# josef-w/Differentiable-iLQR

Measured on AMD Instinct MI355X. Metric: iLQR iters/sec (whole node), batch=65536 cartpole T=25 at 1/2/4/8 MI355X, higher is better.
Workload: dtype f32; 1 GPU; cartpole n=5 m=1 T=25, unconstrained iLQR, 65536 problems per GPU, step = one whole-batch MPC solve of lqr_iter=10 from u=0; batch_per_gpu=65536, global_batch=65536, T=25, lqr_iter=10, parallelism=batch-sharded x1 (no collective)

## Files before the change

### differentiable-ilqr_amd/csrc/dilqr_fused.h

```cpp
#pragma once
#include "dilqr_common.h"
#include "dilqr_launch.h"

namespace dilqr {

constexpr int TRAJ_AOS = 0, TRAJ_REC = 1;

template <int TL, int n, int m>
DEV void ld_xu(float (&x)[n], float (&u)[m], const float* __restrict__ xp, const float* __restrict__ up, size_t t,
               int B, int b) {
  const size_t tb = t * B + b;
  if constexpr (TL == TRAJ_REC) {
    float r[n + m];
    ld(r, (xp + (size_t)b * (n + m)) + t * (size_t)B * (n + m));
#pragma unroll
    for (int i = 0; i < n; ++i) x[i] = r[i];
#pragma unroll
    for (int a = 0; a < m; ++a) u[a] = r[n + a];
  } else {
    ld(x, xp + tb * n);
    ld(u, up + tb * m);
  }
}

template <int TL, int n, int m>
DEV void st_xu(float* __restrict__ xp, float* __restrict__ up, const float (&x)[n], const float (&u)[m], size_t t,
               int B, int b) {
  const size_t tb = t * B + b;
  if constexpr (TL == TRAJ_REC) {
    float r[n + m];
#pragma unroll
    for (int i = 0; i < n; ++i) r[i] = x[i];
#pragma unroll
    for (int a = 0; a < m; ++a) r[n + a] = u[a];
    st(xp + tb * (n + m), r);
  } else {
    st(xp + tb * n, x);
    st(up + tb * m, u);
  }
}

template <int d>
struct CostFull {
  static constexpr bool kDiag = false;
  static constexpr bool kSym = false;
  const float* __restrict__ C;
  const float* __restrict__ c;
  DEV void load(float (&Cr)[d][d], float (&cr)[d], size_t t, int B, int b) const {
    const size_t tb = t * B + b;
    ld2(Cr, C + tb * d * d); ld(cr, c + tb * d);
  }
};

template <int d>
constexpr int packed_cost_floats() { return d * (d + 1) / 2 + d; }
template <int d>
constexpr bool packed_diag_ok() { return (2 * d) % 4 == 0; }

constexpr unsigned char kCostSym = 1, kCostDiag = 2, kCostTinv = 4;

template <int d>
DEV void pack_cost(const float (&C)[d][d], const float (&c)[d], float (&buf)[packed_cost_floats<d>()], bool& sym,
                   bool& diag) {
  int k = 0;
#pragma unroll
  for (int i = 0; i < d; ++i) buf[k++] = C[i][i];
#pragma unroll
  for (int i = 0; i < d; ++i) buf[k++] = c[i];
  unsigned asym = 0u, offd = 0u;
#pragma unroll
  for (int i = 0; i < d; ++i)
#pragma unroll
    for (int j = i + 1; j < d; ++j) {
      asym |= __float_as_uint(C[i][j]) ^ __float_as_uint(C[j][i]);
      offd |= __float_as_uint(C[i][j]) | __float_as_uint(C[j][i]);
      buf[k++] = C[i][j];
    }
  sym &= asym == 0u;
  diag &= offd == 0u;
}

template <int K>
DEV bool same_bits(const float (&a)[K], const float (&b)[K]) {
  unsigned dif = 0u;
#pragma unroll
  for (int k = 0; k < K; ++k) dif |= __float_as_uint(a[k]) ^ __float_as_uint(b[k]);
  return dif == 0u;
}

template <int d, bool DIAG = false, bool TINV = false>
struct CostPacked {
  static constexpr bool kDiag = DIAG;
  static constexpr bool kSym = true;
  const float* __restrict__ P;
  int T;
  DEV void load(float (&Cr)[d][d], float (&cr)[d], size_t t_, int B, int b) const {
    constexpr int PK = packed_cost_floats<d>();
    const size_t t = TINV ? (size_t)(T - 1) : t_;
    if constexpr (DIAG) {
      static_assert(packed_diag_ok<d>(), "diagonal read needs whole float4 planes");
      constexpr int Q4 = SoaRec<PK>::Q4;
      const float4* q = reinterpret_cast<const float4*>(P);
      float buf[2 * d];
#pragma unroll
      for (int j = 0; j < 2 * d / 4; ++j) {
        float4 v = q[(t * Q4 + j) * B + b];
        buf[4 * j] = v.x; buf[4 * j + 1] = v.y; buf[4 * j + 2] = v.z; buf[4 * j + 3] = v.w;
      }
      const float z = 0.f;
#pragma unroll
      for (int i = 0; i < d; ++i) {
#pragma unroll
        for (int j = 0; j < d; ++j) Cr[i][j] = z;
        Cr[i][i] = buf[i];
        cr[i] = buf[d + i];
      }
    } else {
      float buf[PK];
      SoaRec<PK>::load(buf, P, T, t, B, b);
      int k = 2 * d;
#pragma unroll
      for (int i = 0; i < d; ++i) {
        Cr[i][i] = buf[i];
        cr[i] = buf[d + i];
      }
#pragma unroll
      for (int i = 0; i < d; ++i)
#pragma unroll
        for (int j = i + 1; j < d; ++j) { Cr[i][j] = buf[k]; Cr[j][i] = buf[k]; ++k; }
    }
  }
};

template <int d>
struct CostDiagConst {
  static constexpr bool kDiag = true;
  static constexpr bool kSym = true;
  float dg[d], cc[d];
  DEV void init(const float* __restrict__ P, int T, int B, int b) {
    float Cr[d][d], cr[d];
    CostPacked<d, true>{P, T}.load(Cr, cr, T - 1, B, b);
#pragma unroll
    for (int i = 0; i < d; ++i) { dg[i] = Cr[i][i]; cc[i] = cr[i]; }
  }
  template <int PK>
  DEV void set(const float (&pk)[PK]) {
#pragma unroll
    for (int i = 0; i < d; ++i) { dg[i] = pk[i]; cc[i] = pk[d + i]; }
  }
  DEV void load(float (&Cr)[d][d], float (&cr)[d], size_t, int, int) const {
    const float z = 0.f;
#pragma unroll
    for (int i = 0; i < d; ++i) {
#pragma unroll
      for (int j = 0; j < d; ++j) Cr[i][j] = z;
      Cr[i][i] = dg[i];
      cr[i] = cc[i];
    }
  }
};

template <int m, int BM>
struct StepBounds {
  float lo[m], hi[m];
  DEV void load(const Bounds& bd, int t, int B, int b) {
    if constexpr (BM == DILQR_BOUNDS_TENSOR) {
      const size_t tb = (size_t)t * B + b;
      ld(lo, bd.lo_t + tb * m); ld(hi, bd.hi_t + tb * m);
    }
  }
  DEV float l(const Bounds& bd, int a) const {
    if constexpr (BM == DILQR_BOUNDS_TENSOR) return lo[a];
    else return bd.lo;
  }
  DEV float h(const Bounds& bd, int a) const {
    if constexpr (BM == DILQR_BOUNDS_TENSOR) return hi[a];
    else return bd.hi;
  }
};

template <int n, int m, int TL, int BM>
struct SweepIn {
  static constexpr int d = n + m;
  float C[d][d], c[d], x[n], u[m];
  StepBounds<m, BM> bnd;
  template <class CostT>
  DEV void load(const CostT& cs, const float* __restrict__ xp, const float* __restrict__ up, const Bounds& bd, int t,
                int B, int b) {
    cs.load(C, c, t, B, b); ld_xu<TL>(x, u, xp, up, t, B, b); bnd.load(bd, t, B, b);
  }
};

struct GainRecs {
  float* p;
  int B, b;
};

template <int n, int m, int GREC, int TL, int BM>
struct FwdIn {
  static constexpr int d = n + m;
  float g[GREC], u[m], C[d][d], c[d], xnext[n], unext[m];
  StepBounds<m, BM> bnd;
  template <class CostT>
  DEV void load(const GainRecs& gr, const float* __restrict__ up, const CostT& cs,
                const float* __restrict__ xp, const Bounds& bd, int T, int t, int t1, int B, int b) {
    SoaRec<GREC>::load(g, gr.p, T, t, gr.B, gr.b); cs.load(C, c, t, B, b); bnd.load(bd, t, B, b);
    if constexpr (TL == TRAJ_REC) {
      ld_xu<TL>(xnext, unext, xp, up, t1, B, b);
    } else {
      ld(u, up + ((size_t)t * B + b) * m);
      ld(xnext, xp + ((size_t)t1 * B + b) * n);
    }
  }
};

#ifndef DILQR_PF
#define DILQR_PF 2
#endif
constexpr int kPF = DILQR_PF;
#ifndef DILQR_PF_LS
#define DILQR_PF_LS 1
#endif
constexpr int kPFL = DILQR_PF_LS;
static_assert(kPFL == 1 || kPFL == 2, "the line search prefetches one or two steps ahead");

#ifndef DILQR_PHASE_SKIP
#define DILQR_PHASE_SKIP 0
#endif

template <class Model, int BM, int TL, class CostT, bool PAIR = false>
DEV int line_search(int T, int B, int b, const Model md, const float* __restrict__ x_init, const CostT& cs,
                    const float* __restrict__ x, const float* __restrict__ u, const Bounds& bd, float decay,
                    int max_ls, const GainRecs& ws, float* __restrict__ xa_out,
                    float* __restrict__ ua_out, float* __restrict__ xb_out, float* __restrict__ ub_out,
                    float* __restrict__ du_sq, float old_cost, float& cost_out, float& alpha_out,
                    bool b_in_gains = false) {
  constexpr int n = Model::N, m = Model::M, d = n + m;
  constexpr int GREC = m * n + m;
  static_assert(TL != TRAJ_REC || GREC == d, "B records in the gain slots need m = 1");
  if constexpr (PAIR) {
    max_ls = 2;
    b_in_gains = true;
  }
  float alpha = 1.f, cost = 0.f;
  int win = 0;
  for (int p = 0; p < max_ls; p += 2) {
    const bool twoB = p + 1 < max_ls;
    const float aA = alpha, aB = alpha * decay;
    const f2 al = {aA, aB};
    f2 xp[n], dp[n];
    {
      float x0[n];
      ld(x0, x_init + (size_t)b * n);
#pragma unroll
      for (int i = 0; i < n; ++i) { xp[i] = f2{x0[i], x0[i]}; dp[i] = f2{0.f, 0.f}; }
      if constexpr (TL == TRAJ_AOS) {
        st(xa_out + (size_t)b * n, x0);
        if (twoB) st(xb_out + (size_t)b * n, x0);
      }
    }
    f2 cp = {0.f, 0.f};
    auto cl = [T](int s) { return s < T ? s : T - 1; };
    FwdIn<n, m, GREC, TL, BM> cur, n1, n2;
    cur.load(ws, u, cs, x, bd, T, 0, cl(1), B, b);
    if constexpr (TL == TRAJ_REC) {
      float x0r[n];
      ld_xu<TL>(x0r, cur.u, x, u, 0, B, b);
    }
    if constexpr (kPFL >= 2) {
      if (T > 1) n1.load(ws, u, cs, x, bd, T, 1, cl(2), B, b);
    }
    auto step = [&](int t, auto last_c, auto& c, auto& nx) {
      constexpr bool LAST = decltype(last_c)::value;
      if constexpr (!LAST) {
        if constexpr (kPFL >= 2) {
          if (t + 2 < T) n2.load(ws, u, cs, x, bd, T, t + 2, cl(t + 3), B, b);
        } else {
          nx.load(ws, u, cs, x, bd, T, t + 1, cl(t + 2), B, b);
        }
      }
      f2 nu[m];
#pragma unroll
      for (int a = 0; a < m; ++a) {
        f2 sp = {0.f, 0.f};
#pragma unroll
        for (int j = 0; j < n; ++j) sp += c.g[a * n + j] * dp[j];
        nu[a] = (sp + c.u[a]) + al * c.g[m * n + a];
        if constexpr (BM != DILQR_BOUNDS_NONE) {
          const float lo = c.bnd.l(bd, a), hi = c.bnd.h(bd, a);
          nu[a] = f2{eclamp(nu[a].x, lo, hi), eclamp(nu[a].y, lo, hi)};
        }
      }
      {
        float ua[m], ub[m];
#pragma unroll
        for (int a = 0; a < m; ++a) { ua[a] = nu[a].x; ub[a] = nu[a].y; }
        if constexpr (TL == TRAJ_REC) {
          float xa[n], xb[n];
#pragma unroll
          for (int i = 0; i < n; ++i) { xa[i] = xp[i].x; xb[i] = xp[i].y; }
          st_xu<TL>(xa_out, nullptr, xa, ua, t, B, b);
          if (twoB) {
            if (b_in_gains) {
              float rb[d];
#pragma unroll
              for (int i = 0; i < n; ++i) rb[i] = xb[i];
#pragma unroll
              for (int a = 0; a < m; ++a) rb[n + a] = ub[a];
              SoaRec<d>::store(ws.p, rb, T, t, ws.B, ws.b);
            } else {
              st_xu<TL>(xb_out, nullptr, xb, ub, t, B, b);
            }
          }
        } else {
          st(ua_out + ((size_t)t * B + b) * m, ua);
          if (twoB) st(ub_out + ((size_t)t * B + b) * m, ub);
        }
      }
      if (p == 0) {
#pragma unroll
        for (int a = 0; a < m; ++a) {
          float e = c.u[a] - nu[a].x;
          du_sq[((size_t)t * m + a) * B + b] = e * e;
        }
      }
      f2 tau[d];
#pragma unroll
      for (int i = 0; i < n; ++i) tau[i] = xp[i];
#pragma unroll
      for (int a = 0; a < m; ++a) tau[n + a] = nu[a];
      cp += quad_cost<d, CostT::kDiag>(c.C, c.c, tau);
      if constexpr (!LAST) {
        f2 xnext[n];
        md.forward(xp, nu, xnext);
        float xa[n], xb[n];
#pragma unroll
        for (int i = 0; i < n; ++i) {
          dp[i] = xnext[i] - c.xnext[i];
          xp[i] = xnext[i];
          xa[i] = xnext[i].x;
          xb[i] = xnext[i].y;
        }
        if constexpr (TL == TRAJ_AOS) {
          st(xa_out + ((size_t)(t + 1) * B + b) * n, xa);
          if (twoB) st(xb_out + ((size_t)(t + 1) * B + b) * n, xb);
        }
      }
      if constexpr (!LAST) {
        if constexpr (TL == TRAJ_REC) {
#pragma unroll
          for (int a = 0; a < m; ++a) nx.u[a] = c.unext[a];
        }
      }
    };
    for (int t = 0; t < T - 1; ++t) {
      step(t, std::false_type{}, cur, n1);
      cur = n1;
      if constexpr (kPFL >= 2) n1 = n2;
    }
    step(T - 1, std::true_type{}, cur, n1);
    const float cA = cp.x, cB = cp.y;
    if (!(cA > old_cost) || p == max_ls - 1) { cost = cA; alpha = aA; win = 0; break; }
    if (!(cB > old_cost) || p + 1 == max_ls - 1) { cost = cB; alpha = aB; win = 1; break; }
    alpha = aB * decay;
  }
  if constexpr (TL == TRAJ_REC) {
    if (b_in_gains && win == 1) {
      for (int t = 0; t < T; ++t) {
        float rb[d], xt[n], ut[m];
        SoaRec<d>::load(rb, ws.p, T, t, ws.B, ws.b);
#pragma unroll
        for (int i = 0; i < n; ++i) xt[i] = rb[i];
#pragma unroll
        for (int a = 0; a < m; ++a) ut[a] = rb[n + a];
        st_xu<TL>(xb_out, nullptr, xt, ut, t, B, b);
      }
    }
  }
  cost_out = cost;
  alpha_out = alpha;
  return win;
}

template <class Model, int BM, int TL, bool ROLLOUT, class CostT, bool PREV = false>
DEV int ilqr_problem(int T, int B, int b, const Model md, const float* __restrict__ x_init, const CostT& cs,
                     float* __restrict__ pack_out, unsigned char* __restrict__ sym_out, const float* __restrict__ x,
                     const float* __restrict__ u, const Bounds& bd, float decay, int max_ls,
                     const GainRecs& ws, float* __restrict__ xa_out, float* __restrict__ ua_out,
                     float* __restrict__ xb_out, float* __restrict__ ub_out, float* __restrict__ du_sq,
                     float& cost_out, float& alpha_out, bool b_in_gains = false,
                     float prev_cost = 0.f, unsigned* flags_out = nullptr) {
  constexpr int n = Model::N, m = Model::M, d = n + m;
  constexpr int MODE = BM == DILQR_BOUNDS_NONE ? GAIN_UNC : GAIN_BOX;
  constexpr int GREC = m * n + m;
  constexpr int PK = packed_cost_floats<d>();
  float old_cost = 0.f;
  if constexpr (PREV) old_cost = prev_cost;
  bool sym = true, diag = true, tinv = true;
  bool symsofar = true;
  float pk_last[PK];
  {
    RiccatiState<n, m> rs;
    rs.init();
    float xn[n];
#pragma unroll
    for (int i = 0; i < n; ++i) xn[i] = 0.f;
    SweepIn<n, m, TL, BM> cur, n1, n2;
    cur.load(cs, x, u, bd, T - 1, B, b);
    if constexpr (kPF >= 2) n1.load(cs, x, u, bd, T > 1 ? T - 2 : 0, B, b);
    using SI = SweepIn<n, m, TL, BM>;
    auto sweep_body = [&](int t, auto last_c, const SI& cur, float (&g)[GREC]) {
      constexpr bool LAST = decltype(last_c)::value;
      float tau[d], Ctau[d], cb[d];
#pragma unroll
      for (int i = 0; i < n; ++i) tau[i] = cur.x[i];
#pragma unroll
      for (int a = 0; a < m; ++a) tau[n + a] = cur.u[a];
      if (pack_out) {
        float buf[PK];
        pack_cost(cur.C, cur.c, buf, sym, diag);
        if constexpr (LAST) {
          SoaRec<PK>::store(pack_out, buf, T, t, B, b);
#pragma unroll
          for (int k = 0; k < PK; ++k) pk_last[k] = buf[k];
        } else {
          const bool same = same_bits(buf, pk_last);
          if (tinv && !same)
            for (int s = t + 1; s < T - 1; ++s) SoaRec<PK>::store(pack_out, pk_last, T, s, B, b);
          tinv &= same;
          if (!tinv) SoaRec<PK>::store(pack_out, buf, T, t, B, b);
        }
      }
      float obj = 0.f;
      if constexpr (PREV) c_tau<d, CostT::kDiag>(cur.C, tau, Ctau);
      else obj = quad_cost<d, CostT::kDiag>(cur.C, cur.c, tau, Ctau);
#pragma unroll
      for (int i = 0; i < d; ++i) cb[i] = Ctau[i] + cur.c[i];
      float Ft[n][d];
      if constexpr (!LAST) {
        if constexpr (ROLLOUT && Model::kJacFromNext) md.jacobian_next(cur.x, cur.u, xn, Ft);
        else md.jacobian(cur.x, cur.u, Ft);
      } else {
#pragma unroll
        for (int i = 0; i < n; ++i)
#pragma unroll
          for (int j = 0; j < d; ++j) Ft[i][j] = 0.f;
      }
      float zIt[m], lb[m], ub[m];
#pragma unroll
      for (int a = 0; a < m; ++a) {
        zIt[a] = 0.f; lb[a] = 0.f; ub[a] = 0.f;
        if constexpr (MODE == GAIN_BOX) {
          lb[a] = cur.bnd.l(bd, a) - cur.u[a];
          ub[a] = cur.bnd.h(bd, a) - cur.u[a];
        }
      }
      float Kt[m][n], kt[m];
      using FS = typename Model::FSparsity;
      if constexpr (CostT::kSym) {
        rs.template step<MODE, FS, CostT::kDiag, true>(cur.C, cb, Ft, zIt, lb, ub, Kt, kt);
      } else {
        symsofar &= bitwise_symmetric(cur.C);
        if (symsofar) rs.template step<MODE, FS, CostT::kDiag, true>(cur.C, cb, Ft, zIt, lb, ub, Kt, kt);
        else rs.template step<MODE, FS, CostT::kDiag, false>(cur.C, cb, Ft, zIt, lb, ub, Kt, kt);
      }
#pragma unroll
      for (int a = 0; a < m; ++a) {
#pragma unroll
        for (int j = 0; j < n; ++j) g[a * n + j] = Kt[a][j];
        g[m * n + a] = kt[a];
      }
      if constexpr (!PREV) old_cost += obj;
#pragma unroll
      for (int i = 0; i < n; ++i) xn[i] = cur.x[i];
    };
    auto sweep_step = [&](int t, auto last_c) {
      if constexpr (kPF >= 2) n2.load(cs, x, u, bd, t > 1 ? t - 2 : 0, B, b);
      else n1.load(cs, x, u, bd, t > 0 ? t - 1 : 0, B, b);
      float g[GREC];
      sweep_body(t, last_c, cur, g);
      SoaRec<GREC>::store(ws.p, g, T, t, ws.B, ws.b);
      cur = n1;
      if constexpr (kPF >= 2) n1 = n2;
    };
    sweep_step(T - 1, std::true_type{});
#ifndef DILQR_SWEEP_UNROLL
#define DILQR_SWEEP_UNROLL 2
#endif
#pragma unroll DILQR_SWEEP_UNROLL
    for (int t = T - 2; t >= 0; --t) sweep_step(t, std::false_type{});
    if (sym_out) {
      const unsigned char f = sym ? (unsigned char)(kCostSym | (diag && packed_diag_ok<d>() ? kCostDiag : 0) |
                                                    (tinv ? kCostTinv : 0))
                                  : 0;
      sym_out[b] = f;
      if (flags_out) *flags_out = f;
    }
  }
  DILQR_STAMP(2);
#if DILQR_PHASE_SKIP & 1
  cost_out = old_cost;
  alpha_out = 1.f;
  return 0;
#endif
  if constexpr (!CostT::kDiag && packed_diag_ok<d>()) {
    if (pack_out && sym && diag && tinv) {
      CostDiagConst<d> cc;
      cc.set(pk_last);
      if (b_in_gains && max_ls == 2)
        return line_search<Model, BM, TL, CostDiagConst<d>, true>(T, B, b, md, x_init, cc, x, u, bd, decay, max_ls, ws,
                                                                  xa_out, ua_out, xb_out, ub_out, du_sq, old_cost,
                                                                  cost_out, alpha_out, b_in_gains);
      return line_search<Model, BM, TL>(T, B, b, md, x_init, cc, x, u, bd, decay, max_ls, ws, xa_out, ua_out,
                                         xb_out, ub_out, du_sq, old_cost, cost_out, alpha_out, b_in_gains);
    }
  }
  if (b_in_gains && max_ls == 2)
    return line_search<Model, BM, TL, CostT, true>(T, B, b, md, x_init, cs, x, u, bd, decay, max_ls, ws, xa_out,
                                                   ua_out, xb_out, ub_out, du_sq, old_cost, cost_out, alpha_out,
                                                   b_in_gains);
  return line_search<Model, BM, TL>(T, B, b, md, x_init, cs, x, u, bd, decay, max_ls, ws, xa_out, ua_out, xb_out,
                                     ub_out, du_sq, old_cost, cost_out, alpha_out, b_in_gains);
}

template <class Model, int BM>
__global__ void __launch_bounds__(kBlock) k_ilqr_iterate(int T, int B, const float* __restrict__ theta,
                                                         const float* __restrict__ x_init, const float* __restrict__ C,
                                                         const float* __restrict__ c, const float* __restrict__ x,
                                                         const float* __restrict__ u, Bounds bd, float decay, int max_ls,
                                                         float* __restrict__ ws, float* __restrict__ x_out,
                                                         float* __restrict__ u_out, float* __restrict__ cost_out,
                                                         float* __restrict__ du_sq, float* __restrict__ alpha_out,
                                                         const dilqr_mpc_ctrl* __restrict__ ctrl) {
  if (ctrl && ctrl->stopped) return;
  int b = blockIdx.x * blockDim.x + threadIdx.x;
  if (b >= B) return;
  constexpr int n = Model::N, m = Model::M;
  constexpr int GREC = m * n + m;
  Model md; md.load(theta);
  float cost, alpha;
  float* xb = ws + (size_t)T * B * GREC;
  float* ub = xb + (size_t)T * B * n;
  const int win = ilqr_problem<Model, BM, TRAJ_AOS, false>(T, B, b, md, x_init, CostFull<n + m>{C, c}, nullptr, nullptr, x, u,
                                                   bd, decay,
                                            max_ls, GainRecs{ws, B, b},
                                            x_out, u_out, xb, ub, du_sq, cost, alpha);
  if (win) {
    for (int t = 0; t < T; ++t) {
      const size_t tb = (size_t)t * B + b;
      float xt[n], ut[m];
      ld(xt, xb + tb * n); ld(ut, ub + tb * m);
      st(x_out + tb * n, xt); st(u_out + tb * m, ut);
    }
  }
  cost_out[b] = cost;
  alpha_out[b] = alpha;
}

using MpcState = dilqr_mpc_state;
constexpr int kSlots = 4;

DEV bool mpc_decide(const MpcState& S, int B, int k, int G, float eps, int not_improved_lim);

DEV void free_slots(int cur, int best, int& sa, int& sb) {
  sa = -1;
  sb = -1;
#pragma unroll
  for (int s = 0; s < kSlots; ++s) {
    const bool fr = s != cur && s != best;
    sb = (fr && sa >= 0 && sb < 0) ? s : sb;
    sa = (fr && sa < 0) ? s : sa;
  }
}

struct LaneIter {
  float cost, alpha;
  int slot;
};

template <class Model, int BM, bool LG, bool FIRST, bool PREV = true, int GS = kBlock>
DEV LaneIter mpc_iteration_lane(int T, int B, int b, const Model md, const float* __restrict__ x_init,
                                const float* __restrict__ C, const float* __restrict__ c, const Bounds& bd,
                                float decay, int max_ls, const MpcState& S, float* __restrict__ du_sq,
                                float* __restrict__ lds_gains, int cur, int best, unsigned pk, float prev_cost,
                                unsigned* flags_out = nullptr) {
  constexpr int n = Model::N, m = Model::M;
  const size_t TBd = (size_t)T * B * (n + m);
  int sa, sb;
  free_slots(cur, best, sa, sb);
  const float* xcur = S.Xs + cur * TBd;
  float* xsa = S.Xs + sa * TBd;
  float* xsb = S.Xs + sb * TBd;
  float cost, alpha;
  int win;
  const GainRecs gr = LG ? GainRecs{lds_gains, GS, (int)threadIdx.x} : GainRecs{S.ws, B, b};
  const CostFull<n + m> full{C, c};
  const bool b_lds = LG && max_ls <= 2;
  if constexpr (FIRST) {
    win = ilqr_problem<Model, BM, TRAJ_REC, true>(T, B, b, md, x_init, full, S.Cpk, S.Cpk ? S.cost_sym : nullptr,
                                                  xcur, nullptr, bd, decay, max_ls, gr, xsa, nullptr, xsb, nullptr,
                                                  du_sq, cost, alpha, b_lds, 0.f, flags_out);
  } else {
    if ((pk & (kCostDiag | kCostTinv)) == (kCostDiag | kCostTinv)) {
      if constexpr (packed_diag_ok<n + m>()) {
        CostDiagConst<n + m> cc;
        cc.init(S.Cpk, T, B, b);
        win = ilqr_problem<Model, BM, TRAJ_REC, true, CostDiagConst<n + m>, PREV>(T, B, b, md, x_init, cc, nullptr, nullptr, xcur, nullptr, bd,
                                                      decay, max_ls, gr, xsa, nullptr, xsb, nullptr, du_sq, cost,
                                                      alpha, b_lds, prev_cost);
      } else {
        __builtin_unreachable();
      }
#ifdef DILQR_ONLY_DIAGCONST
    } else {
      __builtin_unreachable();
    }
#else
    } else if (pk & kCostDiag) {
      if constexpr (packed_diag_ok<n + m>())
        win = ilqr_problem<Model, BM, TRAJ_REC, true, CostPacked<n + m, true>, PREV>(T, B, b, md, x_init, CostPacked<n + m, true>{S.Cpk, T}, nullptr,
                                                      nullptr, xcur, nullptr, bd, decay, max_ls, gr, xsa, nullptr, xsb,
                                                      nullptr, du_sq, cost, alpha, b_lds, prev_cost);
      else
        __builtin_unreachable();
    } else if ((pk & (kCostSym | kCostTinv)) == (kCostSym | kCostTinv))
      win = ilqr_problem<Model, BM, TRAJ_REC, true, CostPacked<n + m, false, true>, PREV>(T, B, b, md, x_init, CostPacked<n + m, false, true>{S.Cpk, T},
                                                    nullptr, nullptr, xcur, nullptr, bd, decay, max_ls, gr, xsa, nullptr,
                                                    xsb, nullptr, du_sq, cost, alpha, b_lds, prev_cost);
    else if (pk & kCostSym)
      win = ilqr_problem<Model, BM, TRAJ_REC, true, CostPacked<n + m>, PREV>(T, B, b, md, x_init, CostPacked<n + m>{S.Cpk, T}, nullptr, nullptr,
                                                    xcur, nullptr, bd, decay, max_ls, gr, xsa, nullptr, xsb, nullptr,
                                                    du_sq, cost, alpha, b_lds, prev_cost);
    else
      win = ilqr_problem<Model, BM, TRAJ_REC, true, CostFull<n + m>, PREV>(T, B, b, md, x_init, full, nullptr, nullptr, xcur, nullptr, bd,
                                                    decay, max_ls, gr, xsa, nullptr, xsb, nullptr, du_sq, cost,
                                                    alpha, b_lds, prev_cost);
#endif
  }
  return LaneIter{cost, alpha, win ? sb : sa};
}

DEV bool mpc_takes_best(bool first, float cost, float best_cost, float best_cost_eps) {
  return first || cost <= best_cost + best_cost_eps;
}

template <class Model, int BM, bool LG, bool FIRST>
__global__ void __launch_bounds__(kBlock) k_mpc_iterate(int T, int B, const float* __restrict__ theta,
                                                        const float* __restrict__ x_init, const float* __restrict__ C,
                                                        const float* __restrict__ c, Bounds bd, float decay, int max_ls,
                                                        int iteration, float best_cost_eps, float eps,
                                                        int not_improved_lim, int G, MpcState S) {
  constexpr bool first = FIRST;
  int b = blockIdx.x * blockDim.x + threadIdx.x;
  const int bl = b < B ? b : B - 1;
  const int cur = S.slot[bl], best = S.slot[B + bl];
  const unsigned char pk = (!FIRST && S.Cpk) ? S.cost_sym[bl] : 0;
  const float prev = FIRST ? 0.f : S.cost[bl];
  const float best_cost = FIRST ? 0.f : S.best_cost[bl];
  DILQR_STAMP(0);
  DILQR_STAMP(6);
  if (mpc_decide(S, B, iteration, G, eps, not_improved_lim)) return;
  if (b >= B) return;
  DILQR_STAMP(1);
  Model md; md.load(theta);
  extern __shared__ __attribute__((aligned(16))) float lds_gains[];
  const LaneIter r = mpc_iteration_lane<Model, BM, LG, FIRST>(T, B, b, md, x_init, C, c, bd, decay, max_ls, S,
                                                              S.du_sq, lds_gains, cur, best, pk, prev);
  DILQR_STAMP(3);
  S.cost[b] = r.cost;
  S.alpha[b] = r.alpha;
  const bool take = mpc_takes_best(first, r.cost, best_cost, best_cost_eps);
  if (take) {
    S.best_cost[b] = r.cost;
    S.slot[B + b] = (unsigned char)r.slot;
  }
  S.improved[b] = take ? (first ? 1 : 2) : 0;
  if (S.best_iter && take) S.best_iter[b] = iteration;
  S.slot[b] = (unsigned char)r.slot;
  DILQR_STAMP(4);
  DILQR_STAMP(7);
}

DEV int sync_gmax(int B) { return (B + 63) / 64; }

DEV bool mpc_decide(const MpcState& S, int B, int k, int G, float eps, int not_improved_lim) {
  if (k == 0) return false;
  if (G < 0) return false;
  const int gm = sync_gmax(B), par = (k - 1) & 1;
  const unsigned* pm = S.done_counter + 16 + (2 * par) * gm;
  const unsigned* pa = S.done_counter + 16 + (2 * par + 1) * gm;
  const int lane = threadIdx.x & 63;
  const dilqr_mpc_ctrl in = S.ctrl[(k - 1) & 1];
  unsigned mx = 0u;
  int any = 0;
  if ((gm & 3) == 0 && G <= 1024) {
    const uint4* pm4 = reinterpret_cast<const uint4*>(pm);
    const uint4* pa4 = reinterpret_cast<const uint4*>(pa);
    uint4 vm[4], va[4];
#pragma unroll
    for (int j = 0; j < 4; ++j) {
      const int i = lane + 64 * j;
      const bool ok = 4 * i < G;
      vm[j] = ok ? pm4[i] : make_uint4(0u, 0u, 0u, 0u);
      va[j] = ok ? pa4[i] : make_uint4(0u, 0u, 0u, 0u);
    }
#pragma unroll
    for (int j = 0; j < 4; ++j) {
      const int i0 = 4 * (lane + 64 * j);
      const unsigned e[4] = {vm[j].x, vm[j].y, vm[j].z, vm[j].w};
      const unsigned f[4] = {va[j].x, va[j].y, va[j].z, va[j].w};
#pragma unroll
      for (int q = 0; q < 4; ++q) {
        if (i0 + q < G) {
          mx = e[q] > mx ? e[q] : mx;
          any |= (int)f[q];
        }
      }
    }
  } else {
    for (int i = lane; i < G; i += 64) {
      unsigned v = pm[i];
      mx = v > mx ? v : mx;
      any |= (int)pa[i];
    }
  }
  dilqr_mpc_ctrl out = in;
  if (!in.stopped) {
    const bool all_below = __ballot(!(__uint_as_float(mx) < eps)) == 0ull;
    const bool any_imp = __ballot(any != 0) != 0ull;
    out.iter = in.iter + 1;
    out.n_not_improved = any_imp ? 0 : in.n_not_improved + 1;
    if (all_below || out.n_not_improved > not_improved_lim) out.stopped = 1;
    if (blockIdx.x == 0) {
#pragma unroll
      for (int off = 32; off > 0; off >>= 1) {
        unsigned o = __shfl_xor(mx, off, 64);
        mx = o > mx ? o : mx;
      }
      out.max_du_bits = mx;
    }
  }
  if (blockIdx.x == 0 && threadIdx.x == 0) S.ctrl[k & 1] = out;
  return out.stopped != 0;
}

template <class Model>
constexpr int slot_layout() { return Model::N + Model::M <= 8 ? TRAJ_REC : TRAJ_AOS; }
constexpr int slot_layout_nm(int n, int m) { return n + m <= 8 ? TRAJ_REC : TRAJ_AOS; }

#ifndef DILQR_BEGIN_PF
#define DILQR_BEGIN_PF 1
#endif
template <class Model, bool ANALYSE = false>
DEV unsigned mpc_begin_lane(int T, int B, int b, const Model& md, const float* __restrict__ x_init,
                            const float* __restrict__ u_init, const MpcState& S,
                            const float* __restrict__ C = nullptr, const float* __restrict__ c = nullptr) {
  constexpr int n = Model::N, m = Model::M, d = n + m;
  constexpr int PK = packed_cost_floats<d>();
  S.slot[b] = 0; S.slot[B + b] = 0;
  constexpr int TL = slot_layout<Model>();
  const CostFull<d> full{C, c};
  constexpr int PFB = ANALYSE ? DILQR_BEGIN_PF : 1;
  float Cq[PFB][d][d], cq[PFB][d], uq[PFB][m];
  auto load_step = [&](int s, int t) {
    if (u_init) {
      ld(uq[s], u_init + ((size_t)t * B + b) * m);
    } else {
#pragma unroll
      for (int a = 0; a < m; ++a) uq[s][a] = 0.f;
    }
    if constexpr (ANALYSE) full.load(Cq[s], cq[s], t, B, b);
  };
#pragma unroll
  for (int s = 0; s < PFB; ++s) load_step(s, s < T ? s : T - 1);
  bool sym = true, diag = true, tinv = true;
  float pk_first[PK];
  float xt[n];
  ld(xt, x_init + (size_t)b * n);
  for (int t0 = 0; t0 < T; t0 += PFB) {
#pragma unroll
    for (int s = 0; s < PFB; ++s) {
      const int t = t0 + s;
      if (t >= T) break;
      float ut[m], xn[n];
      float Cc[d][d], cc[d];
#pragma unroll
      for (int a = 0; a < m; ++a) ut[a] = uq[s][a];
      if constexpr (ANALYSE) {
#pragma unroll
        for (int i = 0; i < d; ++i) {
          cc[i] = cq[s][i];
#pragma unroll
          for (int j = 0; j < d; ++j) Cc[i][j] = Cq[s][i][j];
        }
      }
      const int tp = t + PFB < T ? t + PFB : T - 1;
      load_step(s, tp);
      st_xu<TL>(S.Xs, S.Us, xt, ut, t, B, b);
      if (t < T - 1) {
        md.forward(xt, ut, xn);
#pragma unroll
        for (int i = 0; i < n; ++i) xt[i] = xn[i];
      }
      if constexpr (ANALYSE) {
        float buf[PK];
        pack_cost(Cc, cc, buf, sym, diag);
        if (t == 0) {
#pragma unroll
          for (int k = 0; k < PK; ++k) pk_first[k] = buf[k];
        } else {
          const bool same = same_bits(buf, pk_first);
          if (tinv && !same)
            for (int s_ = 0; s_ < t; ++s_) SoaRec<PK>::store(S.Cpk, pk_first, T, s_, B, b);
          tinv &= same;
          if (!tinv) SoaRec<PK>::store(S.Cpk, buf, T, t, B, b);
        }
      }
    }
  }
  if constexpr (ANALYSE) {
    if (tinv) SoaRec<PK>::store(S.Cpk, pk_first, T, T - 1, B, b);
    const unsigned char f = sym ? (unsigned char)(kCostSym | (diag && packed_diag_ok<d>() ? kCostDiag : 0) |
                                                  (tinv ? kCostTinv : 0))
                                : 0;
    S.cost_sym[b] = f;
    return f;
  }
  return 0u;
}

constexpr int kDenseCount = 9;

DEV void mpc_reset_ctrl(const MpcState& S) {
  dilqr_mpc_ctrl z = {};
  S.ctrl[0] = z;
  S.ctrl[1] = z;
#pragma unroll
  for (int i = 0; i <= kDenseCount; ++i) S.done_counter[i] = 0u;
}

#ifndef DILQR_SOLVE_LPW
#define DILQR_SOLVE_LPW 64
#endif
#ifndef DILQR_SOLVE_OCC
#define DILQR_SOLVE_OCC 1
#endif
constexpr int kSolveLpw = DILQR_SOLVE_LPW;

template <class Model, int BM, bool LG>
__global__ void __launch_bounds__(kBlock, DILQR_SOLVE_OCC) k_mpc_solve_fixed(int T, int B, const float* __restrict__ theta,
                                                            const float* __restrict__ x_init,
                                                            const float* __restrict__ u_init,
                                                            const float* __restrict__ C, const float* __restrict__ c,
                                                            Bounds bd, float decay, int max_ls, int iters,
                                                            float best_cost_eps, MpcState S) {
  constexpr int m = Model::M;
  const int b = blockIdx.x * kSolveLpw + threadIdx.x;
  DILQR_STAMP(0);
  DILQR_STAMP(6);
  if (b == 0) mpc_reset_ctrl(S);
  if (b >= B || (int)threadIdx.x >= kSolveLpw) return;
  Model md; md.load(theta);
  extern __shared__ __attribute__((aligned(16))) float lds_gains[];
  const unsigned pk = S.Cpk ? mpc_begin_lane<Model, true>(T, B, b, md, x_init, u_init, S, C, c)
                            : mpc_begin_lane<Model>(T, B, b, md, x_init, u_init, S);
  DILQR_STAMP(1);
  LaneIter r = mpc_iteration_lane<Model, BM, LG, false, false, kSolveLpw>(T, B, b, md, x_init, C, c, bd, decay,
                                                                          max_ls, S, S.du_sq, lds_gains, 0, 0, pk,
                                                                          0.f);
  int cur = r.slot, best = r.slot, best_iter = 0;
  float best_cost = r.cost;
  bool take = true;
  DILQR_STAMP(3);
  const size_t plane = (size_t)T * m * B;
  for (int it = 1; it < iters; ++it) {
    if (it == iters - 1) DILQR_STAMP(4);
    r = mpc_iteration_lane<Model, BM, LG, false, true, kSolveLpw>(T, B, b, md, x_init, C, c, bd, decay, max_ls, S,
                                                                  S.du_sq + it * plane, lds_gains, cur, best, pk,
                                                                  r.cost);
    take = mpc_takes_best(false, r.cost, best_cost, best_cost_eps);
    if (take) { best_cost = r.cost; best = r.slot; best_iter = it; }
    cur = r.slot;
  }
  S.cost[b] = r.cost;
  S.alpha[b] = r.alpha;
  S.best_cost[b] = best_cost;
  S.slot[b] = (unsigned char)cur;
  S.slot[B + b] = (unsigned char)best;
  S.improved[b] = take ? (iters == 1 ? 1 : 2) : 0;
  S.best_iter[b] = best_iter;
  DILQR_STAMP(5);
  DILQR_STAMP(7);
}

constexpr int kSmallMax = 256;

template <class Model, int BM, bool LG>
__global__ void __launch_bounds__(kSmallMax) k_mpc_solve_small(int T, int B, const float* __restrict__ theta,
                                                               const float* __restrict__ x_init,
                                                               const float* __restrict__ u_init,
                                                               const float* __restrict__ C,
                                                               const float* __restrict__ c, Bounds bd, float decay,
                                                               int max_ls, int iters, float best_cost_eps, float eps,
                                                               int not_improved_lim, MpcState S) {
  constexpr int m = Model::M;
  __shared__ unsigned red_max[kSmallMax / 64];
  __shared__ int red_any[kSmallMax / 64];
  extern __shared__ __attribute__((aligned(16))) float lds_gains[];
  const int b = threadIdx.x;
  const bool act = b < B;
  const int nw = (int)(blockDim.x + 63) / 64, w = b >> 6;
  const int TM = T * m;
  Model md; md.load(theta);
  unsigned pk = 0u;
  LaneIter r{0.f, 0.f, 0};
  int cur = 0, best = 0, imp = 0;
  float best_cost = 0.f;
  if (act) {
    pk = S.Cpk ? mpc_begin_lane<Model, true>(T, B, b, md, x_init, u_init, S, C, c)
               : mpc_begin_lane<Model>(T, B, b, md, x_init, u_init, S);
    r = mpc_iteration_lane<Model, BM, LG, false, false, 64>(T, B, b, md, x_init, C, c, bd, decay, max_ls, S,
                                                            S.du_sq, lds_gains, 0, 0, pk, 0.f);
    cur = best = r.slot;
    best_cost = r.cost;
    imp = 1;
  }
  int done = 0, n_not_improved = 0, stopped = 0;
  unsigned mx_all = 0u, mx_prev = 0u;
  for (;;) {
    ++done;
    __syncthreads();
    unsigned mx = 0u;
    int any = 0;
    if (act) {
      float s2 = 0.f;
      const float* p = S.du_sq + (size_t)b * TM;
      for (int i = 0; i < TM; ++i) s2 += p[i];
      const float fdn = sqrtf(s2);
      S.full_du_norm[b] = fdn;
      if (imp) S.best_du[b] = fdn;
      mx = __float_as_uint(fdn);
      any = imp == 2;
    }
#pragma unroll
    for (int off = 32; off > 0; off >>= 1) {
      const unsigned o = __shfl_xor(mx, off, 64);
      mx = o > mx ? o : mx;
      any |= __shfl_xor(any, off, 64);
    }
    if ((b & 63) == 0) { red_max[w] = mx; red_any[w] = any; }
    __syncthreads();
    mx = 0u;
    any = 0;
    for (int i = 0; i < nw; ++i) { mx = red_max[i] > mx ? red_max[i] : mx; any |= red_any[i]; }
    mx_prev = mx_all;
    mx_all = mx;
    if (done == iters) break;
    n_not_improved = any ? 0 : n_not_improved + 1;
    if (__uint_as_float(mx) < eps || n_not_improved > not_improved_lim) {
      stopped = 1;
      break;
    }
    if (act) {
      r = mpc_iteration_lane<Model, BM, LG, false, true, 64>(T, B, b, md, x_init, C, c, bd, decay, max_ls, S,
                                                             S.du_sq, lds_gains, cur, best, pk, r.cost);
      const bool take = mpc_takes_best(false, r.cost, best_cost, best_cost_eps);
      if (take) { best_cost = r.cost; best = r.slot; }
      imp = take ? 2 : 0;
      cur = r.slot;
    }
  }
  if (act) {
    S.cost[b] = r.cost;
    S.alpha[b] = r.alpha;
    S.best_cost[b] = best_cost;
    S.slot[b] = (unsigned char)cur;
    S.slot[B + b] = (unsigned char)best;
    S.improved[b] = imp;
  }
  if (b == 0) {
    dilqr_mpc_ctrl o = {};
    o.iter = stopped ? done : done - 1;
    o.stopped = stopped;
    o.n_not_improved = n_not_improved;
    o.max_du_bits = stopped ? mx_all : mx_prev;
    S.ctrl[0] = o;
    S.ctrl[1] = o;
  }
}

inline bool lds_gains_fit(size_t lds, int B) {
  if (kNoLdsGains || lds > 65536) return false;
  if (lds * 4 <= kLdsPerCU) return true;
  static int cus = [] {
    int dev = 0, n = 0;
    if (hipGetDevice(&dev) != hipSuccess ||
        hipDeviceGetAttribute(&n, hipDeviceAttributeMultiprocessorCount, dev) != hipSuccess)
      return 0;
    return n;
  }();
  return (size_t)grid_for(B) <= (size_t)cus * (kLdsPerCU / lds);
}
template <class MD>
int launch_mpc_step_tpp(const MpcStepArgs& a) {
#define LAUNCH_IT(BM_, LG_, FIRST_, LDS_)                                                                     \
  k_mpc_iterate<MD, BM_, LG_, FIRST_><<<grid_for(a.B), kBlock, LDS_, a.stream>>>(                            \
      a.T, a.B, a.theta, a.x_init, a.C, a.c, a.bd, a.decay, a.max_ls, a.iteration, a.best_cost_eps, a.eps, a.lim, \
      a.G, a.st)
#define LAUNCH_MPC(BM_)                                                                                      \
  do {                                                                                                       \
    const size_t lds = (size_t)a.T * kBlock * (MD::N * MD::M + MD::M) * sizeof(float);                      \
    const bool lg = lds_gains_fit(lds, a.B);                                                                 \
    if (a.iteration == 0 && lg) LAUNCH_IT(BM_, true, true, lds);                                             \
    else if (a.iteration == 0) LAUNCH_IT(BM_, false, true, 0);                                               \
    else if (lg) LAUNCH_IT(BM_, true, false, lds);                                                           \
    else LAUNCH_IT(BM_, false, false, 0);                                                                    \
  } while (0)
  if (a.bd.mode == DILQR_BOUNDS_TENSOR) LAUNCH_MPC(DILQR_BOUNDS_TENSOR);
  else if (a.bd.mode != DILQR_BOUNDS_NONE) LAUNCH_MPC(DILQR_BOUNDS_SCALAR);
  else LAUNCH_MPC(DILQR_BOUNDS_NONE);
#undef LAUNCH_MPC
#undef LAUNCH_IT
  return launched();
}

template <class MD>
int launch_mpc_solve_tpp(const MpcSolveArgs& a) {
#define LAUNCH_SOLVE(BM_)                                                                                    \
  do {                                                                                                       \
    const size_t lds = (size_t)a.T * kSolveLpw * (MD::N * MD::M + MD::M) * sizeof(float);                   \
    const int grid = (int)(((long long)a.B + kSolveLpw - 1) / kSolveLpw);                                   \
    if (lds_gains_fit(lds * kBlock / kSolveLpw, a.B))                                                       \
      k_mpc_solve_fixed<MD, BM_, true><<<grid, kBlock, lds, a.stream>>>(                                      \
          a.T, a.B, a.theta, a.x_init, a.u_init, a.C, a.c, a.bd, a.decay, a.max_ls, a.iters, a.best_cost_eps, a.st); \
    else                                                                                                     \
      k_mpc_solve_fixed<MD, BM_, false><<<grid, kBlock, 0, a.stream>>>(                                       \
          a.T, a.B, a.theta, a.x_init, a.u_init, a.C, a.c, a.bd, a.decay, a.max_ls, a.iters, a.best_cost_eps, a.st); \
  } while (0)
  if (a.bd.mode == DILQR_BOUNDS_TENSOR) LAUNCH_SOLVE(DILQR_BOUNDS_TENSOR);
  else if (a.bd.mode != DILQR_BOUNDS_NONE) LAUNCH_SOLVE(DILQR_BOUNDS_SCALAR);
  else LAUNCH_SOLVE(DILQR_BOUNDS_NONE);
#undef LAUNCH_SOLVE
  return launched();
}

template <class MD>
int launch_mpc_solve_small_tpp(const MpcSolveArgs& a, float eps, int lim) {
  if (a.B > kSmallMax) return DILQR_E_SHAPE;
  const int threads = (a.B + 63) / 64 * 64;
  const size_t lds = (size_t)a.T * 64 * (MD::N * MD::M + MD::M) * sizeof(float);
  const bool lg = threads == 64 && lds <= 65536 && !kNoLdsGains;
#define LAUNCH_SMALL(BM_)                                                                                    \
  do {                                                                                                       \
    if (lg)                                                                                                  \
      k_mpc_solve_small<MD, BM_, true><<<1, threads, lds, a.stream>>>(                                        \
          a.T, a.B, a.theta, a.x_init, a.u_init, a.C, a.c, a.bd, a.decay, a.max_ls, a.iters, a.best_cost_eps, eps, \
          lim, a.st);                                                                                        \
    else                                                                                                     \
      k_mpc_solve_small<MD, BM_, false><<<1, threads, 0, a.stream>>>(                                         \
          a.T, a.B, a.theta, a.x_init, a.u_init, a.C, a.c, a.bd, a.decay, a.max_ls, a.iters, a.best_cost_eps, eps, \
          lim, a.st);                                                                                        \
  } while (0)
  if (a.bd.mode == DILQR_BOUNDS_TENSOR) LAUNCH_SMALL(DILQR_BOUNDS_TENSOR);
  else if (a.bd.mode != DILQR_BOUNDS_NONE) LAUNCH_SMALL(DILQR_BOUNDS_SCALAR);
  else LAUNCH_SMALL(DILQR_BOUNDS_NONE);
#undef LAUNCH_SMALL
  return launched();
}

template <class MD>
int launch_ilqr_iterate_tpp(const IlqrIterArgs& a) {
#define LAUNCH_IT(BM_)                                                                                        \
  k_ilqr_iterate<MD, BM_><<<grid_for(a.B), kBlock, 0, a.stream>>>(a.T, a.B, a.theta, a.x_init, a.C, a.c, a.x, a.u, \
                                                                   a.bd, a.decay, a.max_ls, a.ws, a.x_out,     \
                                                                   a.u_out, a.cost, a.du_sq, a.alpha, a.ctrl)
  if (a.bd.mode == DILQR_BOUNDS_TENSOR) LAUNCH_IT(DILQR_BOUNDS_TENSOR);
  else if (a.bd.mode != DILQR_BOUNDS_NONE) LAUNCH_IT(DILQR_BOUNDS_SCALAR);
  else LAUNCH_IT(DILQR_BOUNDS_NONE);
#undef LAUNCH_IT
  return launched();
}

}
```

Baseline: 1.923 billion problem-iters/s.

## Speculate time-invariant diagonal cost from endpoints and verify lazily inside solve

Before solving, each lane checks only the first and last cost timesteps. If both are diagonal, symmetric and identical, it skips the full per-step cost analysis, writes one packed record and runs the specialised diag-const iteration path. The remaining timesteps are checked later, after one iteration chosen per block (blocks spread over up to 8 groups), using batched loads. If that check fails, the lane falls back and reruns the full original path, so a mismatch wastes work and adds code size and register pressure to the kernel.

New measurement: 1.830 billion problem-iters/s. -4.8%, worse.

```diff
diff --git a/differentiable-ilqr_amd/csrc/dilqr_fused.h b/differentiable-ilqr_amd/csrc/dilqr_fused.h
--- a/differentiable-ilqr_amd/csrc/dilqr_fused.h
+++ b/differentiable-ilqr_amd/csrc/dilqr_fused.h
@@ -578,7 +578,7 @@
   int slot;
 };
 
-template <class Model, int BM, bool LG, bool FIRST, bool PREV = true, int GS = kBlock>
+template <class Model, int BM, bool LG, bool FIRST, bool PREV = true, int GS = kBlock, bool ONLY7 = false>
 DEV LaneIter mpc_iteration_lane(int T, int B, int b, const Model md, const float* __restrict__ x_init,
                                 const float* __restrict__ C, const float* __restrict__ c, const Bounds& bd,
                                 float decay, int max_ls, const MpcState& S, float* __restrict__ du_sq,
@@ -601,7 +601,7 @@
                                                   xcur, nullptr, bd, decay, max_ls, gr, xsa, nullptr, xsb, nullptr,
                                                   du_sq, cost, alpha, b_lds, 0.f, flags_out);
   } else {
-    if ((pk & (kCostDiag | kCostTinv)) == (kCostDiag | kCostTinv)) {
+    if (ONLY7 || (pk & (kCostDiag | kCostTinv)) == (kCostDiag | kCostTinv)) {
       if constexpr (packed_diag_ok<n + m>()) {
         CostDiagConst<n + m> cc;
         cc.init(S.Cpk, T, B, b);
@@ -829,6 +829,67 @@
   return 0u;
 }
 
+template <int d>
+DEV bool cost_probe_ends(int T, int B, int b, const float* __restrict__ C, const float* __restrict__ c,
+                         float (&held)[2 * d]) {
+  if constexpr (!packed_diag_ok<d>()) {
+    return false;
+  } else {
+    constexpr int PK = packed_cost_floats<d>();
+    const CostFull<d> full{C, c};
+    float C0[d][d], c0[d], C1[d][d], c1[d];
+    full.load(C0, c0, 0, B, b);
+    full.load(C1, c1, T - 1, B, b);
+    bool sym = true, diag = true;
+    float first[PK], last[PK];
+    pack_cost(C0, c0, first, sym, diag);
+    pack_cost(C1, c1, last, sym, diag);
+#pragma unroll
+    for (int k = 0; k < 2 * d; ++k) held[k] = first[k];
+    return sym && diag && same_bits(first, last);
+  }
+}
+
+template <int d>
+DEV bool is_held_record(const float (&buf)[packed_cost_floats<d>()], bool sym, bool diag, const float (&held)[2 * d]) {
+  unsigned dif = 0u;
+#pragma unroll
+  for (int k = 0; k < 2 * d; ++k) dif |= __float_as_uint(buf[k]) ^ __float_as_uint(held[k]);
+  return sym && diag && dif == 0u;
+}
+
+#ifndef DILQR_SPEC_BATCH
+#define DILQR_SPEC_BATCH 6
+#endif
+constexpr int kSpecBatch = DILQR_SPEC_BATCH;
+
+template <int d>
+DEV bool spec_verify_steps(const CostFull<d>& full, int T, int B, int b, const float (&held)[2 * d]) {
+  constexpr int PK = packed_cost_floats<d>();
+  bool sym = true, diag = true, same = true;
+  for (int t0 = 1; t0 <= T - 2; t0 += kSpecBatch) {
+    float Cq[kSpecBatch][d][d], cq[kSpecBatch][d];
+#pragma unroll
+    for (int j = 0; j < kSpecBatch; ++j) full.load(Cq[j], cq[j], t0 + j <= T - 2 ? t0 + j : T - 1, B, b);
+#pragma unroll
+    for (int j = 0; j < kSpecBatch; ++j) {
+      float buf[PK];
+      pack_cost(Cq[j], cq[j], buf, sym, diag);
+      same &= is_held_record<d>(buf, sym, diag, held);
+    }
+  }
+  return same;
+}
+
+#ifndef DILQR_SPEC_GROUPS
+#define DILQR_SPEC_GROUPS 8
+#endif
+constexpr int kSpecGroups = DILQR_SPEC_GROUPS;
+DEV int spec_verify_after(int iters) {
+  const int groups = iters < kSpecGroups ? (iters < 1 ? 1 : iters) : kSpecGroups;
+  return (int)(blockIdx.x % (unsigned)groups);
+}
+
 constexpr int kDenseCount = 9;
 
 DEV void mpc_reset_ctrl(const MpcState& S) {
@@ -847,6 +908,58 @@
 #endif
 constexpr int kSolveLpw = DILQR_SOLVE_LPW;
 
+struct SolveLane {
+  LaneIter r;
+  int cur, best, best_iter;
+  float best_cost;
+  bool take;
+};
+
+template <class Model, int BM, bool LG>
+DEV bool mpc_solve_speculated(int T, int B, int b, const Model& md, const float* __restrict__ x_init,
+                              const float* __restrict__ u_init, const float* __restrict__ C,
+                              const float* __restrict__ c, const Bounds& bd, float decay, int max_ls, int iters,
+                              float best_cost_eps, const MpcState& S, float* __restrict__ lds_gains,
+                              const float (&held)[2 * (Model::N + Model::M)], SolveLane& out) {
+  constexpr int m = Model::M, d = Model::N + Model::M;
+  constexpr int PK = packed_cost_floats<d>();
+  constexpr unsigned pk = kCostSym | kCostDiag | kCostTinv;
+  const CostFull<d> full{C, c};
+  const int vit = spec_verify_after(iters);
+  mpc_begin_lane<Model>(T, B, b, md, x_init, u_init, S);
+  {
+    float rec[PK];
+#pragma unroll
+    for (int k = 0; k < PK; ++k) rec[k] = 0.f;
+#pragma unroll
+    for (int k = 0; k < 2 * d; ++k) rec[k] = held[k];
+    SoaRec<PK>::store(S.Cpk, rec, T, T - 1, B, b);
+    S.cost_sym[b] = (unsigned char)pk;
+  }
+  DILQR_STAMP(1);
+  LaneIter r = mpc_iteration_lane<Model, BM, LG, false, false, kSolveLpw, true>(T, B, b, md, x_init, C, c, bd, decay,
+                                                                                max_ls, S, S.du_sq, lds_gains, 0, 0,
+                                                                                pk, 0.f);
+  if (vit == 0 && !spec_verify_steps<d>(full, T, B, b, held)) return false;
+  int cur = r.slot, best = r.slot, best_iter = 0;
+  float best_cost = r.cost;
+  bool take = true;
+  DILQR_STAMP(3);
+  const size_t plane = (size_t)T * m * B;
+  for (int it = 1; it < iters; ++it) {
+    if (it == iters - 1) DILQR_STAMP(4);
+    r = mpc_iteration_lane<Model, BM, LG, false, true, kSolveLpw, true>(T, B, b, md, x_init, C, c, bd, decay, max_ls,
+                                                                        S, S.du_sq + it * plane, lds_gains, cur, best,
+                                                                        pk, r.cost);
+    if (vit == it && !spec_verify_steps<d>(full, T, B, b, held)) return false;
+    take = mpc_takes_best(false, r.cost, best_cost, best_cost_eps);
+    if (take) { best_cost = r.cost; best = r.slot; best_iter = it; }
+    cur = r.slot;
+  }
+  out = SolveLane{r, cur, best, best_iter, best_cost, take};
+  return true;
+}
+
 template <class Model, int BM, bool LG>
 __global__ void __launch_bounds__(kBlock, DILQR_SOLVE_OCC) k_mpc_solve_fixed(int T, int B, const float* __restrict__ theta,
                                                             const float* __restrict__ x_init,
@@ -854,7 +967,7 @@
                                                             const float* __restrict__ C, const float* __restrict__ c,
                                                             Bounds bd, float decay, int max_ls, int iters,
                                                             float best_cost_eps, MpcState S) {
-  constexpr int m = Model::M;
+  constexpr int n = Model::N, m = Model::M, d = n + m;
   const int b = blockIdx.x * kSolveLpw + threadIdx.x;
   DILQR_STAMP(0);
   DILQR_STAMP(6);
@@ -862,26 +975,41 @@
   if (b >= B || (int)threadIdx.x >= kSolveLpw) return;
   Model md; md.load(theta);
   extern __shared__ __attribute__((aligned(16))) float lds_gains[];
-  const unsigned pk = S.Cpk ? mpc_begin_lane<Model, true>(T, B, b, md, x_init, u_init, S, C, c)
-                            : mpc_begin_lane<Model>(T, B, b, md, x_init, u_init, S);
-  DILQR_STAMP(1);
-  LaneIter r = mpc_iteration_lane<Model, BM, LG, false, false, kSolveLpw>(T, B, b, md, x_init, C, c, bd, decay,
-                                                                          max_ls, S, S.du_sq, lds_gains, 0, 0, pk,
-                                                                          0.f);
-  int cur = r.slot, best = r.slot, best_iter = 0;
-  float best_cost = r.cost;
-  bool take = true;
-  DILQR_STAMP(3);
-  const size_t plane = (size_t)T * m * B;
-  for (int it = 1; it < iters; ++it) {
-    if (it == iters - 1) DILQR_STAMP(4);
-    r = mpc_iteration_lane<Model, BM, LG, false, true, kSolveLpw>(T, B, b, md, x_init, C, c, bd, decay, max_ls, S,
-                                                                  S.du_sq + it * plane, lds_gains, cur, best, pk,
-                                                                  r.cost);
-    take = mpc_takes_best(false, r.cost, best_cost, best_cost_eps);
-    if (take) { best_cost = r.cost; best = r.slot; best_iter = it; }
-    cur = r.slot;
-  }
+  SolveLane sl;
+  bool done = false;
+  if constexpr (packed_diag_ok<d>()) {
+    float held[2 * d];
+    if (S.Cpk && cost_probe_ends<d>(T, B, b, C, c, held))
+      done = mpc_solve_speculated<Model, BM, LG>(T, B, b, md, x_init, u_init, C, c, bd, decay, max_ls, iters,
+                                                 best_cost_eps, S, lds_gains, held, sl);
+  }
+  if (!done) {
+    const unsigned pk = S.Cpk ? mpc_begin_lane<Model, true>(T, B, b, md, x_init, u_init, S, C, c)
+                              : mpc_begin_lane<Model>(T, B, b, md, x_init, u_init, S);
+    DILQR_STAMP(1);
+    LaneIter r = mpc_iteration_lane<Model, BM, LG, false, false, kSolveLpw>(T, B, b, md, x_init, C, c, bd, decay,
+                                                                            max_ls, S, S.du_sq, lds_gains, 0, 0, pk,
+                                                                            0.f);
+    int cur = r.slot, best = r.slot, best_iter = 0;
+    float best_cost = r.cost;
+    bool take = true;
+    DILQR_STAMP(3);
+    const size_t plane = (size_t)T * m * B;
+    for (int it = 1; it < iters; ++it) {
+      if (it == iters - 1) DILQR_STAMP(4);
+      r = mpc_iteration_lane<Model, BM, LG, false, true, kSolveLpw>(T, B, b, md, x_init, C, c, bd, decay, max_ls, S,
+                                                                    S.du_sq + it * plane, lds_gains, cur, best, pk,
+                                                                    r.cost);
+      take = mpc_takes_best(false, r.cost, best_cost, best_cost_eps);
+      if (take) { best_cost = r.cost; best = r.slot; best_iter = it; }
+      cur = r.slot;
+    }
+    sl = SolveLane{r, cur, best, best_iter, best_cost, take};
+  }
+  const LaneIter r = sl.r;
+  const int cur = sl.cur, best = sl.best, best_iter = sl.best_iter;
+  const float best_cost = sl.best_cost;
+  const bool take = sl.take;
   S.cost[b] = r.cost;
   S.alpha[b] = r.alpha;
   S.best_cost[b] = best_cost;
```
